# april-tools/cirkit

Hardware: AMD Instinct MI355X
Metric: log-likelihood evals/sec (batch 4096 per GPU) on 784-var QuadTree PC (higher is better)
Workload: dtype f32

## Files before the change

### cirkit_amd/csrc/ck_tailp.hip

```cpp
#include <algorithm>

#include "ck_internal.h"
#include "ck_softmax.h"
#include "ck_tailwalk.h"

namespace {

constexpr int kRowsPerBlock = 4;

struct TailParamsArgs {
  const TailFold* folds;
  const int32_t* level_begin;
  TailWalkArgs walk;
  const int32_t* bad_input;
  int n_slots;
  int n_tail;
  const float* cat_logits;
  const int64_t* cat_idx;
  const float* dense_logits;
  float* table;
  float* scale;
  int n_tables, C;
  int n_pair;
  const ck_rows32_job* rows;
  int n_rows;
#ifdef CK_TAILP_STAMPS
  long long* stamps;
#endif
};

#ifdef CK_TAILP_STAMPS
#define CK_TP_STAMP(k)                                                                                          \
  do {                                                                                                          \
    if (a.stamps != nullptr && threadIdx.x == 0) a.stamps[16 * blockIdx.x + (k)] = static_cast<long long>(wall_clock64()); \
  } while (0)
#else
#define CK_TP_STAMP(k)
#endif

__global__ void __launch_bounds__(512, 4) tail_params_kernel(const TailParamsArgs a) {
  extern __shared__ __attribute__((aligned(16))) float smem[];
  const int lane = threadIdx.x & 63;
  const int wave = __builtin_amdgcn_readfirstlane(threadIdx.x >> 6);
  const int bid = blockIdx.x;
  CK_TP_STAMP(0);
  if (bid < a.n_tail) {
    TailFold* s_fold = reinterpret_cast<TailFold*>(smem);
    int32_t* s_level = reinterpret_cast<int32_t*>(s_fold + a.walk.n_folds);
    float* tiles_base = smem + kTailCtlFloats;
    {
      const int n16 = a.walk.n_folds * static_cast<int>(sizeof(TailFold) / 16);
      const int4* src = reinterpret_cast<const int4*>(a.folds);
      int4* dst = reinterpret_cast<int4*>(s_fold);
      for (int i = threadIdx.x; i < n16; i += blockDim.x) dst[i] = src[i];
      for (int i = threadIdx.x; i <= a.walk.n_levels; i += blockDim.x) s_level[i] = a.level_begin[i];
    }
    __syncthreads();
    const bool poison = a.bad_input != nullptr && *a.bad_input != 0;
    const TailTiles tiles{tiles_base, tiles_base, a.n_slots};
#ifdef CK_TAILP_STAMPS
    g_tail_level_stamps = a.stamps != nullptr ? a.stamps + 16 * blockIdx.x + 2 : nullptr;
#endif
    CK_TP_STAMP(1);
    tail_walk<8, false>(a.walk, bid, tiles, s_fold, s_level, poison, wave, WorkgroupBarrier{});
    CK_TP_STAMP(15);
    return;
  }
  const int v = bid - a.n_tail;
  if (v < a.n_pair) {
    const int half = wave >> 2, w4 = wave & 3, kh = lane >> 5;
    const int C = a.C;
    float* tile = smem + half * (32 * (C + 4) + 1024);
    const int d = 2 * v + half;
    const float *theta = nullptr, *theta_w = nullptr;
    if (d < a.n_tables) {
      const int64_t f = a.cat_idx != nullptr ? a.cat_idx[d] : d;
      theta = a.cat_logits + f * 32 * C;
      theta_w = a.dense_logits + static_cast<int64_t>(d) * 1024;
    }
    float* dst = a.table + static_cast<int64_t>(d) * (C + 1) * 32;
    float* dsc = a.scale + static_cast<int64_t>(d) * (C + 1);
    table_dense_rows<4, true>(theta, theta_w, C, tile, w4, lane, [] { __syncthreads(); }, [&](int c, const float (&val)[16], float m) {
      if (c <= C && kh == 0) dsc[c] = m;
      if (c <= C) tile_store(dst + static_cast<int64_t>(c) * 32 + 4 * kh, val);
    });
    CK_TP_STAMP(15);
    return;
  }
  const int x0 = (v - a.n_pair) * kRowsPerBlock;
  const int n = min(kRowsPerBlock, a.n_rows - x0);
  ck_rows32_job xj[kRowsPerBlock];
#pragma unroll
  for (int i = 0; i < kRowsPerBlock; ++i) xj[i] = a.rows[x0 + min(i, n - 1)];
  float xr[kRowsPerBlock][2];
#pragma unroll
  for (int i = 0; i < kRowsPerBlock; ++i) softmax_rows32_load<2>(xj[i].in, xj[i].rows, wave, 8, lane, xr[i]);
#pragma unroll
  for (int i = 0; i < kRowsPerBlock; ++i) {
    if (i < n) {
      float* const out = xj[i].out;
      const bool tiled = xj[i].tiled != 0;
      softmax_rows32_apply<2>(xr[i], xj[i].rows, wave, 8, lane, [&](int row, int l, float p) { ck::as_global(out)[w32_index(row, l, tiled)] = p; });
    }
  }
  CK_TP_STAMP(15);
}

}

extern "C" int ck_tail_params_fwd(const ck_tail_params_launch* d, void* stream) {
  CK_REQUIRE(d != nullptr, "ck_tail_params_fwd: null descriptor");
  CK_REQUIRE(d->folds && d->level_begin && d->n_folds > 0 && d->n_levels > 0 && d->n_levels <= 15 && d->B > 0,
             "ck_tail_params_fwd: bad tail description");
  CK_REQUIRE(ck::aligned16(d->folds), "ck_tail_params_fwd: folds not 16-byte aligned");
  CK_REQUIRE(d->ll == nullptr || (d->ll_partial != nullptr && d->ll_ticket != nullptr), "ck_tail_params_fwd: ll needs ll_partial and ll_ticket");
  CK_REQUIRE(d->w_layout == CK_W_TILED_F32 || d->w_layout == CK_W_ROWMAJOR, "ck_tail_params_fwd: tail weights must be CK_W_TILED_F32 or row-major");
  CK_REQUIRE(d->n_tables == 0 || (d->cat_logits && d->dense_logits && d->table && d->table_scale), "ck_tail_params_fwd: table jobs need "
             "cat_logits, dense_logits, table and table_scale");
  CK_REQUIRE(d->n_tables == 0 || (d->C > 0 && d->C <= 256 && (d->C & 3) == 0), "ck_tail_params_fwd: table jobs need C <= 256, C %% 4 == 0");
  CK_REQUIRE(d->n_rows == 0 || d->rows != nullptr, "ck_tail_params_fwd: rows is null");
  const size_t ctl = static_cast<size_t>(d->n_folds) * sizeof(TailFold) + (d->n_levels + 1) * sizeof(int32_t);
  const size_t lds_tail = kTailCtlFloats * sizeof(float) + static_cast<size_t>(d->n_slots) * 2048;
  const size_t lds_pair = d->n_tables > 0 ? static_cast<size_t>(2) * (32 * (d->C + 4) + 1024) * sizeof(float) : 0;
  const size_t lds = std::max(lds_tail, lds_pair);
  if (ctl > kTailCtlFloats * sizeof(float) || d->n_slots <= 0 || lds > 80 * 1024)
    return ck::fail(CK_ERR_UNSUPPORTED, "ck_tail_params_fwd: %d folds in %d slots do not fit two blocks per compute unit", d->n_folds, d->n_slots);
  TailParamsArgs a{};
  a.folds = reinterpret_cast<const TailFold*>(d->folds);
  a.level_begin = d->level_begin;
  a.walk.B = d->B;
  a.walk.n_levels = d->n_levels;
  a.walk.n_folds = d->n_folds;
  a.walk.w_rowmajor = d->w_layout == CK_W_ROWMAJOR ? 1 : 0;
  a.walk.write = 1;
  a.walk.ll = d->ll;
  a.walk.ll_partial = d->ll_partial;
  a.walk.ll_ticket = d->ll_ticket;
  a.bad_input = d->bad_input;
  a.n_slots = d->n_slots;
  a.n_tail = (d->B + 15) / 16;
  a.cat_logits = d->cat_logits;
  a.cat_idx = d->cat_idx;
  a.dense_logits = d->dense_logits;
  a.table = d->table;
  a.scale = d->table_scale;
  a.n_tables = d->n_tables;
  a.C = d->C;
  a.n_pair = (d->n_tables + 1) / 2;
  a.rows = d->rows;
  a.n_rows = d->n_rows;
#ifdef CK_TAILP_STAMPS
  a.stamps = getenv("CK_STAMP_PTR") != nullptr ? reinterpret_cast<long long*>(strtoull(getenv("CK_STAMP_PTR"), nullptr, 0)) : nullptr;
#endif
  const int blocks = a.n_tail + a.n_pair + (d->n_rows + kRowsPerBlock - 1) / kRowsPerBlock;
  const TailParamsArgs a0 = a;
  const void* const* ll_slot = nullptr;
  if (d->ll_cell != 0) {
    CK_REQUIRE(d->ll != nullptr, "ck_tail_params_fwd: ll_cell=%d without ll (the pair's home while the cell is NULL)", d->ll_cell);
    ll_slot = ck::program_input_slot(d->ll_cell);
    CK_REQUIRE(d->ll_cell > 0 && ll_slot != nullptr, "ck_tail_params_fwd: ll_cell=%d names a program input, but no program is being "
               "recorded on this thread (or the index is outside 1..%d)", d->ll_cell, ck::kProgramInputs - 1);
  }
  return ck::dispatch(
      [=](hipStream_t s) {
        TailParamsArgs a = a0;
        if (ll_slot != nullptr && *ll_slot != nullptr) a.walk.ll = static_cast<double*>(const_cast<void*>(*ll_slot));
        if (lds > 48 * 1024) {
          hipError_t e = hipFuncSetAttribute(reinterpret_cast<const void*>(tail_params_kernel), hipFuncAttributeMaxDynamicSharedMemorySize,
                                             static_cast<int>(lds));
          if (e != hipSuccess) return e;
        }
        hipLaunchKernelGGL(tail_params_kernel, dim3(blocks), dim3(512), lds, s, a);
        return hipGetLastError();
      },
      stream);
}
```

### cirkit_amd/csrc/ck_tailwalk.h

```cpp
#pragma once

#include "ck_internal.h"
#include "ck_tile.h"
#include "ck_tile16.h"

namespace {

struct TailFold {
  const float* w;
  float* out;
  const float* child[4];
  int32_t child_src[4];
  int32_t H, Ko;
  int32_t skip_store;
  int32_t slot;
};
static_assert(sizeof(TailFold) == sizeof(ck_tail16_fold), "TailFold mirrors ck_tail16_fold");

typedef unsigned int u32x4v __attribute__((ext_vector_type(4)));
constexpr int kAuxWriteThrough = 17;
__device__ __forceinline__ __amdgpu_buffer_rsrc_t wt_buffer(const void* uniform_base) {
  return __builtin_amdgcn_make_buffer_rsrc(const_cast<void*>(uniform_base), 0, 0x7fffffff, 0x27000);
}
__device__ __forceinline__ void store4_wt(__amdgpu_buffer_rsrc_t r, uint32_t byte_off, float x, float y, float z, float w) {
  const u32x4v v = {__float_as_uint(x), __float_as_uint(y), __float_as_uint(z), __float_as_uint(w)};
  __builtin_amdgcn_raw_buffer_store_b128(v, r, byte_off, 0, kAuxWriteThrough);
}
__device__ __forceinline__ f32x4v load4_wt(__amdgpu_buffer_rsrc_t r, uint32_t byte_off) {
  const u32x4v v = __builtin_amdgcn_raw_buffer_load_b128(r, byte_off, 0, kAuxWriteThrough);
  return f32x4v{__uint_as_float(v.x), __uint_as_float(v.y), __uint_as_float(v.z), __uint_as_float(v.w)};
}
__device__ __forceinline__ void tile_store_wt(const float* uniform_block, uint32_t row_byte_off, const float (&v)[16]) {
  const __amdgpu_buffer_rsrc_t r = wt_buffer(uniform_block);
#pragma unroll
  for (int g = 0; g < 4; ++g) store4_wt(r, row_byte_off + 32 * g, v[4 * g + 0], v[4 * g + 1], v[4 * g + 2], v[4 * g + 3]);
}


constexpr int kTailCtlFloats = 2048;
struct TailTiles {
  float* main;
  float* more;
  int n_main;
  __device__ __forceinline__ float* of(int t) const { return t < n_main ? main + t * 512 : more + (t - n_main) * 512; }
};

struct TailWalkArgs {
  int B, n_levels, n_folds;
  int w_rowmajor;
  int write;
  double* ll;
  double* ll_partial;
  unsigned int* ll_ticket;
};

struct WorkgroupBarrier {
  __device__ __forceinline__ void operator()() const { asm volatile("s_waitcnt lgkmcnt(0)\n\ts_barrier" ::: "memory"); }
};
struct WaveGroupBarrier {
  unsigned int* ctr;
  unsigned int n;
  unsigned int round;
  __device__ __forceinline__ void operator()() {
    asm volatile("s_waitcnt lgkmcnt(0)" ::: "memory");
    ++round;
    if ((threadIdx.x & 63) == 0) {
      __hip_atomic_fetch_add(ctr, 1u, __ATOMIC_RELAXED, __HIP_MEMORY_SCOPE_WORKGROUP);
      while (__hip_atomic_load(ctr, __ATOMIC_RELAXED, __HIP_MEMORY_SCOPE_WORKGROUP) < round * n) __builtin_amdgcn_s_sleep(1);
    }
    asm volatile("" ::: "memory");
  }
};

#ifdef CK_TAILP_STAMPS
__shared__ long long* g_tail_level_stamps;
#endif
template <int WAVES, bool WT, class Barrier>
__device__ __forceinline__ void tail_walk(const TailWalkArgs& a, int tile, const TailTiles& tiles, const TailFold* s_fold,
                                          const int32_t* s_level, bool poison, int wave, Barrier&& barrier) {
  const int lane = threadIdx.x & 63;
  const int b_in = lane & 15, kq = lane >> 4;
  const int b = tile * 16 + b_in;
  const bool live = b < a.B;
  const int bl = live ? b : a.B - 1;
  const uint32_t row_off = static_cast<uint32_t>(bl * kK + 4 * kq) * 4u;
  struct Children {
    f32x4v m[4][2];
  };
  auto fetch = [&](int t, Children& c) {
#pragma unroll
    for (int h = 0; h < 4; ++h) {
      if (h < s_fold[t].H && s_fold[t].child_src[h] < 0) {
        const uint64_t p = reinterpret_cast<uint64_t>(s_fold[t].child[h]);
        const uint32_t p_lo = static_cast<uint32_t>(__builtin_amdgcn_readfirstlane(static_cast<int>(static_cast<uint32_t>(p))));
        const uint32_t p_hi = static_cast<uint32_t>(__builtin_amdgcn_readfirstlane(static_cast<int>(static_cast<uint32_t>(p >> 32))));
        const uint64_t pu = (static_cast<uint64_t>(p_hi) << 32) | p_lo;
        const __amdgpu_buffer_rsrc_t r = wt_buffer(reinterpret_cast<const void*>(pu));
        if constexpr (WT) {
          c.m[h][0] = load4_wt(r, row_off);
          c.m[h][1] = load4_wt(r, row_off + 64);
        } else {
          const float* row = reinterpret_cast<const float*>(pu) + (row_off >> 2);
          const float4 x0 = ck::gload4(row), x1 = ck::gload4(row + 16);
          c.m[h][0] = f32x4v{x0.x, x0.y, x0.z, x0.w};
          c.m[h][1] = f32x4v{x1.x, x1.y, x1.z, x1.w};
        }
      }
    }
  };
  auto load_w = [&](int t, WRegs16& w) {
    if (s_fold[t].Ko == kK) {
      if (a.w_rowmajor) load_w16<CK_W_ROWMAJOR>(s_fold[t].w, lane, w);
      else load_w16<CK_W_TILED_F32>(s_fold[t].w, lane, w);
    }
  };
  auto first_fold_from = [&](int li) {
    for (; li < a.n_levels; ++li)
      if (s_level[li] + wave < s_level[li + 1]) return s_level[li] + wave;
    return -1;
  };
  WRegs16 w, wn;
  {
    const int t0 = first_fold_from(0);
    if (t0 >= 0) load_w(t0, w);
  }
  for (int li = 0; li < a.n_levels; ++li) {
    const int t1 = s_level[li + 1];
    int t = s_level[li] + wave;
    Children cur, nxt;
    if (t < t1) fetch(t, cur);
    for (; t < t1; t += WAVES) {
      if (t + WAVES < t1) fetch(t + WAVES, nxt);
      const int t_next = t + WAVES < t1 ? t + WAVES : first_fold_from(li + 1);
      if (t_next >= 0) load_w(t_next, wn);
      const int H = s_fold[t].H, Ko = s_fold[t].Ko;
      float v[8];
#pragma unroll
      for (int j = 0; j < 8; ++j) v[j] = 0.f;
#pragma unroll
      for (int h = 0; h < 4; ++h) {
        if (h >= H) break;
        const int src = s_fold[t].child_src[h];
        if (src >= 0) {
          const float* tl = tiles.of(src) + lane * 4;
#pragma unroll
          for (int beta = 0; beta < 2; ++beta) {
            const float4 t4 = *reinterpret_cast<const float4*>(tl + beta * 256);
            v[4 * beta + 0] += t4.x;
            v[4 * beta + 1] += t4.y;
            v[4 * beta + 2] += t4.z;
            v[4 * beta + 3] += t4.w;
          }
        } else {
#pragma unroll
          for (int beta = 0; beta < 2; ++beta)
#pragma unroll
            for (int r = 0; r < 4; ++r) v[4 * beta + r] += cur.m[h][beta][r];
        }
      }
      float* out = s_fold[t].out;
      if (Ko == kK) {
        sum_step16(w, v);
        if (a.write && live && s_fold[t].skip_store == 0) tile16_store(out + static_cast<int64_t>(b) * kK + 4 * kq, v);
        float* tl = tiles.of(s_fold[t].slot) + lane * 4;
#pragma unroll
        for (int beta = 0; beta < 2; ++beta)
          *reinterpret_cast<float4*>(tl + beta * 256) = make_float4(v[4 * beta + 0], v[4 * beta + 1], v[4 * beta + 2], v[4 * beta + 3]);
      } else {
        const float* wf = s_fold[t].w;
        const float m = ck::clamp_finite(row_max8(v));
        const float nml = exp_offset(m, 0.f);
#pragma unroll
        for (int j = 0; j < 8; ++j) v[j] = __builtin_amdgcn_exp2f(fmaf(v[j], kL2E, nml));
        for (int o = 0; o < Ko; ++o) {
          const float* wrow = wf + o * kK + 4 * kq;
          float acc = 0.f;
#pragma unroll
          for (int beta = 0; beta < 2; ++beta) {
            const float4 w4 = ck::gload4(wrow + 16 * beta);
            acc = fmaf(w4.x, v[4 * beta + 0], acc);
            acc = fmaf(w4.y, v[4 * beta + 1], acc);
            acc = fmaf(w4.z, v[4 * beta + 2], acc);
            acc = fmaf(w4.w, v[4 * beta + 3], acc);
          }
          acc = xquad_sum(acc);
          float y = fmaf(__builtin_amdgcn_logf(acc), kLN2, m);
          if (poison) y = __builtin_nanf("");
          if (live && kq == 0) ck::as_global(out)[static_cast<int64_t>(b) * Ko + o] = y;
          if (a.ll != nullptr && t == a.n_folds - 1) {
            double sacc = 0.0;
            for (int r = 0; r < 16; ++r) {
              const float yr = __shfl(y, r, 64);
              if (tile * 16 + r < a.B) sacc += static_cast<double>(yr);
            }
            const unsigned int n_tiles = static_cast<unsigned int>((a.B + 15) >> 4);
            unsigned int ticket = 0;
            if (lane == 0) {
              __hip_atomic_store(a.ll_partial + tile, sacc, __ATOMIC_RELAXED, __HIP_MEMORY_SCOPE_AGENT);
              asm volatile("s_waitcnt vmcnt(0)" ::: "memory");
              ticket = __hip_atomic_fetch_add(a.ll_ticket, 1u, __ATOMIC_RELAXED, __HIP_MEMORY_SCOPE_AGENT);
            }
            ticket = __shfl(ticket, 0, 64);
            if (ticket == n_tiles - 1) {
              double tot = 0.0;
              const __amdgpu_buffer_rsrc_t rp = wt_buffer(a.ll_partial);
              for (unsigned int g0 = 0; g0 < n_tiles; g0 += 256) {
                typedef unsigned int u32x2v __attribute__((ext_vector_type(2)));
                u32x2v pv[4];
#pragma unroll
                for (int k = 0; k < 4; ++k) {
                  const unsigned int g = g0 + lane + 64 * k;
                  pv[k] = g < n_tiles ? __builtin_amdgcn_raw_buffer_load_b64(rp, g * 8u, 0, kAuxWriteThrough) : u32x2v{0u, 0u};
                }
#pragma unroll
                for (int k = 0; k < 4; ++k)
                  if (g0 + lane + 64 * k < n_tiles) tot += __longlong_as_double(static_cast<long long>((static_cast<unsigned long long>(pv[k].y) << 32) | pv[k].x));
              }
#pragma unroll
              for (int off = 32; off > 0; off >>= 1) tot += __shfl_xor(tot, off, 64);
              if (lane == 0) {
                a.ll[0] = tot;
                a.ll[1] = static_cast<double>(a.B);
                __hip_atomic_store(a.ll_ticket, 0u, __ATOMIC_RELAXED, __HIP_MEMORY_SCOPE_AGENT);
              }
            }
          }
        }
      }
      cur = nxt;
      w = wn;
    }
    barrier();
#ifdef CK_TAILP_STAMPS
    if (threadIdx.x == 0 && g_tail_level_stamps != nullptr && li < 12) g_tail_level_stamps[li] = static_cast<long long>(wall_clock64());
#endif
  }
}


}
```

Baseline: 40.82 million.

## Preload upper-level tail weights before final barrier and drop write-through tile paths

The tail walk now detects up to four top levels whose folds fit one per wave and read only LDS children. For those levels it issues every weight load up front, before the last generic-level barrier, so later levels no longer wait on global weight fetches one level at a time. The first narrow weight row is passed in pre-loaded as well. The change also removes the unused write-through and two-pool tile variants, switches to 32-bit byte offsets with a new B limit check, and adds an env var to force the generic path. Holding four weight register sets at once raises register pressure.

```diff
diff --git a/cirkit_amd/csrc/ck_tailp.hip b/cirkit_amd/csrc/ck_tailp.hip
--- a/cirkit_amd/csrc/ck_tailp.hip
+++ b/cirkit_amd/csrc/ck_tailp.hip
@@ -57,12 +57,12 @@
     }
     __syncthreads();
     const bool poison = a.bad_input != nullptr && *a.bad_input != 0;
-    const TailTiles tiles{tiles_base, tiles_base, a.n_slots};
+    const TailTiles tiles{tiles_base};
 #ifdef CK_TAILP_STAMPS
     g_tail_level_stamps = a.stamps != nullptr ? a.stamps + 16 * blockIdx.x + 2 : nullptr;
 #endif
     CK_TP_STAMP(1);
-    tail_walk<8, false>(a.walk, bid, tiles, s_fold, s_level, poison, wave, WorkgroupBarrier{});
+    tail_walk<8>(a.walk, bid, tiles, s_fold, s_level, poison, wave, WorkgroupBarrier{});
     CK_TP_STAMP(15);
     return;
   }
@@ -113,6 +113,7 @@
   CK_REQUIRE(d->folds && d->level_begin && d->n_folds > 0 && d->n_levels > 0 && d->n_levels <= 15 && d->B > 0,
              "ck_tail_params_fwd: bad tail description");
   CK_REQUIRE(ck::aligned16(d->folds), "ck_tail_params_fwd: folds not 16-byte aligned");
+  CK_REQUIRE(d->B < (1 << 25), "ck_tail_params_fwd: B=%d: a (B, 32) block must stay below 4 GiB (32-bit byte offsets)", d->B);
   CK_REQUIRE(d->ll == nullptr || (d->ll_partial != nullptr && d->ll_ticket != nullptr), "ck_tail_params_fwd: ll needs ll_partial and ll_ticket");
   CK_REQUIRE(d->w_layout == CK_W_TILED_F32 || d->w_layout == CK_W_ROWMAJOR, "ck_tail_params_fwd: tail weights must be CK_W_TILED_F32 or row-major");
   CK_REQUIRE(d->n_tables == 0 || (d->cat_logits && d->dense_logits && d->table && d->table_scale), "ck_tail_params_fwd: table jobs need "
@@ -133,6 +134,10 @@
   a.walk.n_folds = d->n_folds;
   a.walk.w_rowmajor = d->w_layout == CK_W_ROWMAJOR ? 1 : 0;
   a.walk.write = 1;
+  {
+    const char* g = getenv("CK_TAIL_WALK_GENERIC");
+    a.walk.phases = g != nullptr && g[0] != '\0' && g[0] != '0' ? 0 : 1;
+  }
   a.walk.ll = d->ll;
   a.walk.ll_partial = d->ll_partial;
   a.walk.ll_ticket = d->ll_ticket;
diff --git a/cirkit_amd/csrc/ck_tailwalk.h b/cirkit_amd/csrc/ck_tailwalk.h
--- a/cirkit_amd/csrc/ck_tailwalk.h
+++ b/cirkit_amd/csrc/ck_tailwalk.h
@@ -17,38 +17,22 @@
 };
 static_assert(sizeof(TailFold) == sizeof(ck_tail16_fold), "TailFold mirrors ck_tail16_fold");
 
-typedef unsigned int u32x4v __attribute__((ext_vector_type(4)));
 constexpr int kAuxWriteThrough = 17;
 __device__ __forceinline__ __amdgpu_buffer_rsrc_t wt_buffer(const void* uniform_base) {
   return __builtin_amdgcn_make_buffer_rsrc(const_cast<void*>(uniform_base), 0, 0x7fffffff, 0x27000);
 }
-__device__ __forceinline__ void store4_wt(__amdgpu_buffer_rsrc_t r, uint32_t byte_off, float x, float y, float z, float w) {
-  const u32x4v v = {__float_as_uint(x), __float_as_uint(y), __float_as_uint(z), __float_as_uint(w)};
-  __builtin_amdgcn_raw_buffer_store_b128(v, r, byte_off, 0, kAuxWriteThrough);
-}
-__device__ __forceinline__ f32x4v load4_wt(__amdgpu_buffer_rsrc_t r, uint32_t byte_off) {
-  const u32x4v v = __builtin_amdgcn_raw_buffer_load_b128(r, byte_off, 0, kAuxWriteThrough);
-  return f32x4v{__uint_as_float(v.x), __uint_as_float(v.y), __uint_as_float(v.z), __uint_as_float(v.w)};
-}
-__device__ __forceinline__ void tile_store_wt(const float* uniform_block, uint32_t row_byte_off, const float (&v)[16]) {
-  const __amdgpu_buffer_rsrc_t r = wt_buffer(uniform_block);
-#pragma unroll
-  for (int g = 0; g < 4; ++g) store4_wt(r, row_byte_off + 32 * g, v[4 * g + 0], v[4 * g + 1], v[4 * g + 2], v[4 * g + 3]);
-}
-
 
 constexpr int kTailCtlFloats = 2048;
 struct TailTiles {
-  float* main;
-  float* more;
-  int n_main;
-  __device__ __forceinline__ float* of(int t) const { return t < n_main ? main + t * 512 : more + (t - n_main) * 512; }
+  float* base;
+  __device__ __forceinline__ float* of(int slot) const { return base + slot * 512; }
 };
 
 struct TailWalkArgs {
   int B, n_levels, n_folds;
   int w_rowmajor;
   int write;
+  int phases;
   double* ll;
   double* ll_partial;
   unsigned int* ll_ticket;
@@ -57,185 +41,252 @@
 struct WorkgroupBarrier {
   __device__ __forceinline__ void operator()() const { asm volatile("s_waitcnt lgkmcnt(0)\n\ts_barrier" ::: "memory"); }
 };
-struct WaveGroupBarrier {
-  unsigned int* ctr;
-  unsigned int n;
-  unsigned int round;
-  __device__ __forceinline__ void operator()() {
-    asm volatile("s_waitcnt lgkmcnt(0)" ::: "memory");
-    ++round;
-    if ((threadIdx.x & 63) == 0) {
-      __hip_atomic_fetch_add(ctr, 1u, __ATOMIC_RELAXED, __HIP_MEMORY_SCOPE_WORKGROUP);
-      while (__hip_atomic_load(ctr, __ATOMIC_RELAXED, __HIP_MEMORY_SCOPE_WORKGROUP) < round * n) __builtin_amdgcn_s_sleep(1);
-    }
-    asm volatile("" ::: "memory");
-  }
-};
 
 #ifdef CK_TAILP_STAMPS
 __shared__ long long* g_tail_level_stamps;
 #endif
-template <int WAVES, bool WT, class Barrier>
+#define CK_TW_INLINE __attribute__((always_inline))
+
+template <int WAVES, class Barrier>
 __device__ __forceinline__ void tail_walk(const TailWalkArgs& a, int tile, const TailTiles& tiles, const TailFold* s_fold,
                                           const int32_t* s_level, bool poison, int wave, Barrier&& barrier) {
+  constexpr int kUpper = 4;
   const int lane = threadIdx.x & 63;
   const int b_in = lane & 15, kq = lane >> 4;
   const int b = tile * 16 + b_in;
   const bool live = b < a.B;
   const int bl = live ? b : a.B - 1;
   const uint32_t row_off = static_cast<uint32_t>(bl * kK + 4 * kq) * 4u;
+  auto at = [](const float* uniform_base, uint32_t byte_off) CK_TW_INLINE {
+    return reinterpret_cast<const float*>(reinterpret_cast<const char*>(uniform_base) + byte_off);
+  };
+
+  const uint32_t woff = 4u * static_cast<uint32_t>(a.w_rowmajor ? w16_offset<CK_W_ROWMAJOR>(lane, 0) : w16_offset<CK_W_TILED_F32>(lane, 0));
+  const int w_dbeta = a.w_rowmajor ? 16 * kK : 64, w_dg = a.w_rowmajor ? 16 : 512;
+
+  int U = a.n_levels;
   struct Children {
     f32x4v m[4][2];
   };
-  auto fetch = [&](int t, Children& c) {
-#pragma unroll
-    for (int h = 0; h < 4; ++h) {
-      if (h < s_fold[t].H && s_fold[t].child_src[h] < 0) {
-        const uint64_t p = reinterpret_cast<uint64_t>(s_fold[t].child[h]);
-        const uint32_t p_lo = static_cast<uint32_t>(__builtin_amdgcn_readfirstlane(static_cast<int>(static_cast<uint32_t>(p))));
-        const uint32_t p_hi = static_cast<uint32_t>(__builtin_amdgcn_readfirstlane(static_cast<int>(static_cast<uint32_t>(p >> 32))));
-        const uint64_t pu = (static_cast<uint64_t>(p_hi) << 32) | p_lo;
-        const __amdgpu_buffer_rsrc_t r = wt_buffer(reinterpret_cast<const void*>(pu));
-        if constexpr (WT) {
-          c.m[h][0] = load4_wt(r, row_off);
-          c.m[h][1] = load4_wt(r, row_off + 64);
-        } else {
-          const float* row = reinterpret_cast<const float*>(pu) + (row_off >> 2);
-          const float4 x0 = ck::gload4(row), x1 = ck::gload4(row + 16);
-          c.m[h][0] = f32x4v{x0.x, x0.y, x0.z, x0.w};
-          c.m[h][1] = f32x4v{x1.x, x1.y, x1.z, x1.w};
-        }
-      }
-    }
-  };
-  auto load_w = [&](int t, WRegs16& w) {
+  auto uniform_ptr = [&](const float* q) CK_TW_INLINE {
+    const uint64_t p = reinterpret_cast<uint64_t>(q);
+    const uint32_t p_lo = static_cast<uint32_t>(__builtin_amdgcn_readfirstlane(static_cast<int>(static_cast<uint32_t>(p))));
+    const uint32_t p_hi = static_cast<uint32_t>(__builtin_amdgcn_readfirstlane(static_cast<int>(static_cast<uint32_t>(p >> 32))));
+    return reinterpret_cast<const float*>((static_cast<uint64_t>(p_hi) << 32) | p_lo);
+  };
+  auto child_row = [&](int t, int h) CK_TW_INLINE { return at(uniform_ptr(s_fold[t].child[h]), row_off); };
+  auto load_child = [&](const float* row, f32x4v (&c)[2]) CK_TW_INLINE {
+    const float4 x0 = ck::gload4(row), x1 = ck::gload4(row + 16);
+    c[0] = f32x4v{x0.x, x0.y, x0.z, x0.w};
+    c[1] = f32x4v{x1.x, x1.y, x1.z, x1.w};
+  };
+  auto fetch = [&](int t, Children& c) CK_TW_INLINE {
+#pragma unroll
+    for (int h = 0; h < 4; ++h)
+      if (h < s_fold[t].H && s_fold[t].child_src[h] < 0) load_child(child_row(t, h), c.m[h]);
+  };
+  auto load_w = [&](int t, WRegs16& w) CK_TW_INLINE {
     if (s_fold[t].Ko == kK) {
-      if (a.w_rowmajor) load_w16<CK_W_ROWMAJOR>(s_fold[t].w, lane, w);
-      else load_w16<CK_W_TILED_F32>(s_fold[t].w, lane, w);
-    }
-  };
-  auto first_fold_from = [&](int li) {
-    for (; li < a.n_levels; ++li)
+      const float* wf = uniform_ptr(s_fold[t].w);
+#pragma unroll
+      for (int bg = 0; bg < 4; ++bg) w.q[bg] = ck::gload4(at(wf + ((bg >> 1) * w_dbeta + (bg & 1) * w_dg), woff));
+    }
+  };
+  auto first_fold_from = [&](int li) CK_TW_INLINE {
+    for (; li < U; ++li)
       if (s_level[li] + wave < s_level[li + 1]) return s_level[li] + wave;
     return -1;
   };
-  WRegs16 w, wn;
-  {
-    const int t0 = first_fold_from(0);
-    if (t0 >= 0) load_w(t0, w);
-  }
-  for (int li = 0; li < a.n_levels; ++li) {
-    const int t1 = s_level[li + 1];
-    int t = s_level[li] + wave;
-    Children cur, nxt;
-    if (t < t1) fetch(t, cur);
-    for (; t < t1; t += WAVES) {
-      if (t + WAVES < t1) fetch(t + WAVES, nxt);
-      const int t_next = t + WAVES < t1 ? t + WAVES : first_fold_from(li + 1);
-      if (t_next >= 0) load_w(t_next, wn);
-      const int H = s_fold[t].H, Ko = s_fold[t].Ko;
-      float v[8];
-#pragma unroll
-      for (int j = 0; j < 8; ++j) v[j] = 0.f;
-#pragma unroll
-      for (int h = 0; h < 4; ++h) {
-        if (h >= H) break;
-        const int src = s_fold[t].child_src[h];
-        if (src >= 0) {
-          const float* tl = tiles.of(src) + lane * 4;
-#pragma unroll
-          for (int beta = 0; beta < 2; ++beta) {
-            const float4 t4 = *reinterpret_cast<const float4*>(tl + beta * 256);
-            v[4 * beta + 0] += t4.x;
-            v[4 * beta + 1] += t4.y;
-            v[4 * beta + 2] += t4.z;
-            v[4 * beta + 3] += t4.w;
+  auto add_lds_child = [&](int slot, float (&v)[8]) CK_TW_INLINE {
+    const float* tl = tiles.of(slot) + lane * 4;
+#pragma unroll
+    for (int beta = 0; beta < 2; ++beta) {
+      const float4 t4 = *reinterpret_cast<const float4*>(tl + beta * 256);
+      v[4 * beta + 0] += t4.x;
+      v[4 * beta + 1] += t4.y;
+      v[4 * beta + 2] += t4.z;
+      v[4 * beta + 3] += t4.w;
+    }
+  };
+  auto add_reg_child = [&](const f32x4v (&c)[2], float (&v)[8]) CK_TW_INLINE {
+#pragma unroll
+    for (int beta = 0; beta < 2; ++beta)
+#pragma unroll
+      for (int r = 0; r < 4; ++r) v[4 * beta + r] += c[beta][r];
+  };
+  auto out_row = [&](int t) CK_TW_INLINE { return const_cast<float*>(at(uniform_ptr(s_fold[t].out), row_off)); };
+  auto finish32 = [&](int t, const WRegs16& w, float (&v)[8]) CK_TW_INLINE {
+    sum_step16(w, v);
+    if (a.write && live && s_fold[t].skip_store == 0) tile16_store(out_row(t), v);
+    float* tl = tiles.of(s_fold[t].slot) + lane * 4;
+#pragma unroll
+    for (int beta = 0; beta < 2; ++beta)
+      *reinterpret_cast<float4*>(tl + beta * 256) = make_float4(v[4 * beta + 0], v[4 * beta + 1], v[4 * beta + 2], v[4 * beta + 3]);
+  };
+  auto finish_narrow = [&](int t, float (&v)[8], bool pre, const float4& p0, const float4& p1) CK_TW_INLINE {
+    const int Ko = s_fold[t].Ko;
+    float* out = s_fold[t].out;
+    const float* wf = uniform_ptr(s_fold[t].w);
+    const float m = ck::clamp_finite(row_max8(v));
+    const float nml = exp_offset(m, 0.f);
+#pragma unroll
+    for (int j = 0; j < 8; ++j) v[j] = __builtin_amdgcn_exp2f(fmaf(v[j], kL2E, nml));
+    for (int o = 0; o < Ko; ++o) {
+      const float* wrow = at(wf + o * kK, 16u * kq);
+      float acc = 0.f;
+#pragma unroll
+      for (int beta = 0; beta < 2; ++beta) {
+        const float4 w4 = pre && o == 0 ? (beta == 0 ? p0 : p1) : ck::gload4(wrow + 16 * beta);
+        acc = fmaf(w4.x, v[4 * beta + 0], acc);
+        acc = fmaf(w4.y, v[4 * beta + 1], acc);
+        acc = fmaf(w4.z, v[4 * beta + 2], acc);
+        acc = fmaf(w4.w, v[4 * beta + 3], acc);
+      }
+      acc = xquad_sum(acc);
+      float y = fmaf(__builtin_amdgcn_logf(acc), kLN2, m);
+      if (poison) y = __builtin_nanf("");
+      if (live && kq == 0) ck::as_global(out)[static_cast<int64_t>(row_off >> 7) * Ko + o] = y;
+      if (a.ll != nullptr && t == a.n_folds - 1) {
+        double sacc = 0.0;
+        for (int r = 0; r < 16; ++r) {
+          const float yr = __shfl(y, r, 64);
+          if (tile * 16 + r < a.B) sacc += static_cast<double>(yr);
+        }
+        const unsigned int n_tiles = static_cast<unsigned int>((a.B + 15) >> 4);
+        unsigned int ticket = 0;
+        if (lane == 0) {
+          __hip_atomic_store(a.ll_partial + tile, sacc, __ATOMIC_RELAXED, __HIP_MEMORY_SCOPE_AGENT);
+          asm volatile("s_waitcnt vmcnt(0)" ::: "memory");
+          ticket = __hip_atomic_fetch_add(a.ll_ticket, 1u, __ATOMIC_RELAXED, __HIP_MEMORY_SCOPE_AGENT);
+        }
+        ticket = __shfl(ticket, 0, 64);
+        if (ticket == n_tiles - 1) {
+          double tot = 0.0;
+          const __amdgpu_buffer_rsrc_t rp = wt_buffer(a.ll_partial);
+          for (unsigned int g0 = 0; g0 < n_tiles; g0 += 256) {
+            typedef unsigned int u32x2v __attribute__((ext_vector_type(2)));
+            u32x2v pv[4];
+#pragma unroll
+            for (int k = 0; k < 4; ++k) {
+              const unsigned int g = g0 + lane + 64 * k;
+              pv[k] = g < n_tiles ? __builtin_amdgcn_raw_buffer_load_b64(rp, g * 8u, 0, kAuxWriteThrough) : u32x2v{0u, 0u};
+            }
+#pragma unroll
+            for (int k = 0; k < 4; ++k)
+              if (g0 + lane + 64 * k < n_tiles) tot += __longlong_as_double(static_cast<long long>((static_cast<unsigned long long>(pv[k].y) << 32) | pv[k].x));
           }
-        } else {
-#pragma unroll
-          for (int beta = 0; beta < 2; ++beta)
-#pragma unroll
-            for (int r = 0; r < 4; ++r) v[4 * beta + r] += cur.m[h][beta][r];
-        }
-      }
-      float* out = s_fold[t].out;
-      if (Ko == kK) {
-        sum_step16(w, v);
-        if (a.write && live && s_fold[t].skip_store == 0) tile16_store(out + static_cast<int64_t>(b) * kK + 4 * kq, v);
-        float* tl = tiles.of(s_fold[t].slot) + lane * 4;
-#pragma unroll
-        for (int beta = 0; beta < 2; ++beta)
-          *reinterpret_cast<float4*>(tl + beta * 256) = make_float4(v[4 * beta + 0], v[4 * beta + 1], v[4 * beta + 2], v[4 * beta + 3]);
-      } else {
-        const float* wf = s_fold[t].w;
-        const float m = ck::clamp_finite(row_max8(v));
-        const float nml = exp_offset(m, 0.f);
-#pragma unroll
-        for (int j = 0; j < 8; ++j) v[j] = __builtin_amdgcn_exp2f(fmaf(v[j], kL2E, nml));
-        for (int o = 0; o < Ko; ++o) {
-          const float* wrow = wf + o * kK + 4 * kq;
-          float acc = 0.f;
-#pragma unroll
-          for (int beta = 0; beta < 2; ++beta) {
-            const float4 w4 = ck::gload4(wrow + 16 * beta);
-            acc = fmaf(w4.x, v[4 * beta + 0], acc);
-            acc = fmaf(w4.y, v[4 * beta + 1], acc);
-            acc = fmaf(w4.z, v[4 * beta + 2], acc);
-            acc = fmaf(w4.w, v[4 * beta + 3], acc);
+#pragma unroll
+          for (int off = 32; off > 0; off >>= 1) tot += __shfl_xor(tot, off, 64);
+          if (lane == 0) {
+            a.ll[0] = tot;
+            a.ll[1] = static_cast<double>(a.B);
+            __hip_atomic_store(a.ll_ticket, 0u, __ATOMIC_RELAXED, __HIP_MEMORY_SCOPE_AGENT);
           }
-          acc = xquad_sum(acc);
-          float y = fmaf(__builtin_amdgcn_logf(acc), kLN2, m);
-          if (poison) y = __builtin_nanf("");
-          if (live && kq == 0) ck::as_global(out)[static_cast<int64_t>(b) * Ko + o] = y;
-          if (a.ll != nullptr && t == a.n_folds - 1) {
-            double sacc = 0.0;
-            for (int r = 0; r < 16; ++r) {
-              const float yr = __shfl(y, r, 64);
-              if (tile * 16 + r < a.B) sacc += static_cast<double>(yr);
-            }
-            const unsigned int n_tiles = static_cast<unsigned int>((a.B + 15) >> 4);
-            unsigned int ticket = 0;
-            if (lane == 0) {
-              __hip_atomic_store(a.ll_partial + tile, sacc, __ATOMIC_RELAXED, __HIP_MEMORY_SCOPE_AGENT);
-              asm volatile("s_waitcnt vmcnt(0)" ::: "memory");
-              ticket = __hip_atomic_fetch_add(a.ll_ticket, 1u, __ATOMIC_RELAXED, __HIP_MEMORY_SCOPE_AGENT);
-            }
-            ticket = __shfl(ticket, 0, 64);
-            if (ticket == n_tiles - 1) {
-              double tot = 0.0;
-              const __amdgpu_buffer_rsrc_t rp = wt_buffer(a.ll_partial);
-              for (unsigned int g0 = 0; g0 < n_tiles; g0 += 256) {
-                typedef unsigned int u32x2v __attribute__((ext_vector_type(2)));
-                u32x2v pv[4];
-#pragma unroll
-                for (int k = 0; k < 4; ++k) {
-                  const unsigned int g = g0 + lane + 64 * k;
-                  pv[k] = g < n_tiles ? __builtin_amdgcn_raw_buffer_load_b64(rp, g * 8u, 0, kAuxWriteThrough) : u32x2v{0u, 0u};
-                }
-#pragma unroll
-                for (int k = 0; k < 4; ++k)
-                  if (g0 + lane + 64 * k < n_tiles) tot += __longlong_as_double(static_cast<long long>((static_cast<unsigned long long>(pv[k].y) << 32) | pv[k].x));
-              }
-#pragma unroll
-              for (int off = 32; off > 0; off >>= 1) tot += __shfl_xor(tot, off, 64);
-              if (lane == 0) {
-                a.ll[0] = tot;
-                a.ll[1] = static_cast<double>(a.B);
-                __hip_atomic_store(a.ll_ticket, 0u, __ATOMIC_RELAXED, __HIP_MEMORY_SCOPE_AGENT);
-              }
-            }
-          }
-        }
-      }
-      cur = nxt;
-      w = wn;
-    }
+        }
+      }
+    }
+  };
+  auto level_done = [&](int li) CK_TW_INLINE {
     barrier();
 #ifdef CK_TAILP_STAMPS
     if (threadIdx.x == 0 && g_tail_level_stamps != nullptr && li < 12) g_tail_level_stamps[li] = static_cast<long long>(wall_clock64());
 #endif
+  };
+
+  {
+    WRegs16 w, wn;
+    const int t_first = s_level[0] + wave < s_level[1] ? s_level[0] + wave : -1;
+    if (t_first >= 0) load_w(t_first, w);
+    if (a.phases != 0) {
+      static_assert(kUpper * WAVES <= 64, "one lane per (candidate level, fold)");
+      const int k = lane / WAVES, i = lane % WAVES, li = a.n_levels - 1 - k;
+      bool ok = true;
+      if (k < kUpper && li >= 1) {
+        const int t0 = s_level[li], n = s_level[li + 1] - t0;
+        ok = n <= WAVES;
+        if (ok && i < n) {
+#pragma unroll
+          for (int h = 0; h < 4; ++h) ok = ok && !(h < s_fold[t0 + i].H && s_fold[t0 + i].child_src[h] < 0);
+        }
+      }
+      const unsigned long long bad = __ballot(ok ? 0 : 1);
+#pragma unroll
+      for (int kk = 0; kk < kUpper; ++kk)
+        if (U == a.n_levels - kk && U > 1 && ((bad >> (kk * WAVES)) & ((1ull << WAVES) - 1)) == 0) --U;
+    }
+    if (t_first < 0) {
+      const int t0 = first_fold_from(1);
+      if (t0 >= 0) load_w(t0, w);
+    }
+    for (int li = 0; li < U; ++li) {
+      if (li > 0) level_done(li - 1);
+      const int t1 = s_level[li + 1];
+      int t = s_level[li] + wave;
+      Children cur, nxt;
+      if (t < t1) fetch(t, cur);
+      for (; t < t1; t += WAVES) {
+        if (t + WAVES < t1) fetch(t + WAVES, nxt);
+        const int t_next = t + WAVES < t1 ? t + WAVES : first_fold_from(li + 1);
+        if (t_next >= 0) load_w(t_next, wn);
+        const int H = s_fold[t].H;
+        float v[8];
+#pragma unroll
+        for (int j = 0; j < 8; ++j) v[j] = 0.f;
+#pragma unroll
+        for (int h = 0; h < 4; ++h) {
+          if (h >= H) break;
+          const int src = s_fold[t].child_src[h];
+          if (src >= 0) add_lds_child(src, v);
+          else add_reg_child(cur.m[h], v);
+        }
+        if (s_fold[t].Ko == kK) finish32(t, w, v);
+        else finish_narrow(t, v, false, float4{}, float4{});
+        cur = nxt;
+        w = wn;
+      }
+    }
+  }
+
+  WRegs16 wu[kUpper];
+  __builtin_amdgcn_s_waitcnt(0x0F70);
+#pragma unroll
+  for (int i = 0; i < kUpper; ++i) {
+    if (U + i < a.n_levels) {
+      const int t = s_level[U + i] + wave;
+      if (t < s_level[U + i + 1]) {
+        if (s_fold[t].Ko == kK) {
+          load_w(t, wu[i]);
+        } else {
+          const float* wrow = at(uniform_ptr(s_fold[t].w), 16u * kq);
+          wu[i].q[0] = ck::gload4(wrow);
+          wu[i].q[1] = ck::gload4(wrow + 16);
+        }
+      }
+    }
+  }
+  level_done(U - 1);
+#pragma unroll
+  for (int i = 0; i < kUpper; ++i) {
+    if (U + i < a.n_levels) {
+      const int t = s_level[U + i] + wave;
+      if (t < s_level[U + i + 1]) {
+        const int H = s_fold[t].H;
+        float v[8];
+#pragma unroll
+        for (int j = 0; j < 8; ++j) v[j] = 0.f;
+#pragma unroll
+        for (int h = 0; h < 4; ++h) {
+          if (h >= H) break;
+          add_lds_child(s_fold[t].child_src[h], v);
+        }
+        if (s_fold[t].Ko == kK) finish32(t, wu[i], v);
+        else finish_narrow(t, v, true, wu[i].q[0], wu[i].q[1]);
+      }
+      level_done(U + i);
+    }
   }
 }
+#undef CK_TW_INLINE
 
 
 }
```

After: 40.50 million. About the same (-0.8%).
